# matteofox/MC-ALF

Measured on AMD Instinct MI355X. Metric: component-pixel Voigt evals/s (sum_s ncomp_s * npix / t), logL batch on MI355X: `value` with the inputs resident in HBM when the timed region starts, `value_host_api` through the host-pointer entry with P in and logL out inside every step, higher is better.
Workload: dtype f64

## Files before the change

mc-alf_amd/csrc/kernels.hip:

```cpp
#include <hip/hip_runtime.h>

#include <cmath>

#include "kernel_args.h"
#include "voigt_device.h"

namespace mcalf {

__device__ __forceinline__ int xcd_raw() { return (int)(__builtin_amdgcn_s_getreg((3 << 11) | 20) & 15); }
__device__ __forceinline__ int xcd_id() { return (int)(__builtin_amdgcn_s_getreg((3 << 11) | 20) & (kXcds - 1)); }

__device__ __forceinline__ int tile_pos(int i) { return (i & 7) * kPlaneStride + (i >> 3); }

template <int kCtrl, int kRowMask = 0xF>
__device__ __forceinline__ double dpp_move(double v) {
    const unsigned long long u = __builtin_bit_cast(unsigned long long, v);
    const int lo = __builtin_amdgcn_update_dpp(0, (int)(unsigned)u, kCtrl, kRowMask, 0xF, false);
    const int hi = __builtin_amdgcn_update_dpp(0, (int)(unsigned)(u >> 32), kCtrl, kRowMask, 0xF, false);
    return __builtin_bit_cast(double, ((unsigned long long)(unsigned)hi << 32) | (unsigned)lo);
}

__device__ __forceinline__ double wave_sum_to_last(double v) {
    v += dpp_move<0x111>(v);
    v += dpp_move<0x112>(v);
    v += dpp_move<0x114>(v);
    v += dpp_move<0x118>(v);
    v += dpp_move<0x142, 0xA>(v);
    v += dpp_move<0x143, 0xC>(v);
    return v;
}

__device__ __forceinline__ double wave_sum(double v) {
#pragma unroll
    for (int off = 32; off > 0; off >>= 1) v += __shfl_down(v, off, 64);
    return v;
}

__device__ __forceinline__ unsigned long long uniform64(unsigned long long v) {
    const unsigned lo = __builtin_amdgcn_readfirstlane((unsigned)v);
    const unsigned hi = __builtin_amdgcn_readfirstlane((unsigned)(v >> 32));
    return ((unsigned long long)hi << 32) | lo;
}

__device__ __forceinline__ double wave_allsum(double v) {
    const unsigned long long u = __builtin_bit_cast(unsigned long long, wave_sum_to_last(v));
    const unsigned lo = __builtin_amdgcn_readlane((unsigned)u, 63), hi = __builtin_amdgcn_readlane((unsigned)(u >> 32), 63);
    return __builtin_bit_cast(double, ((unsigned long long)hi << 32) | lo);
}

__device__ __forceinline__ double block_sum(double v, double* scratch, int tid) {
    v = wave_sum(v);
    if ((tid & 63) == 0) scratch[tid >> 6] = v;
    __syncthreads();
    double s = 0.0;
#pragma unroll
    for (int w = 0; w < kWaves; ++w) s += scratch[w];
    __syncthreads();
    return s;
}

__device__ __forceinline__ double finalize_value(int mode, double sum, double nnz, bool asymm, double c4,
                                                 double c5, double veto4, double veto5) {
    if (mode == kModeChi2) return (nnz == 0.0) ? INFINITY : sum;
    if (asymm && (c5 > veto5 || c4 > veto4)) return -INFINITY;
    return -0.5 * sum;
}

__device__ __noinline__ double pow10_edge(double x) { return pow(10.0, x); }
__device__ __forceinline__ double pow10_fast(double x) {
    constexpr double kLn10Hi = 2.302585092994045901, kLn10Lo = -2.1707562233822494e-16;
    if (!(fabs(x) <= 300.0)) return pow10_edge(x);
    const double p = x * kLn10Hi;
    const double e = fma(x, kLn10Hi, -p) + x * kLn10Lo;
    const double r = exp_neg(-p);
    return fma(r, e, r);
}

__device__ inline void build_line_record(double* rec, double logN, double z, double b_kms, const LineDev& ln,
                                         double dnu_seg) {
    const double cold = pow10_fast(logN);
    const double zp1 = z + 1.0;
    const double rdnu = ln.wrest_cm / (b_kms * 1e5);
    const double a = ln.gamma4pi * rdnu;
    const double cne = kTauConst * cold * ln.f;
    const double K = cne * rdnu;
    rec[0] = zp1 * rdnu;
    rec[1] = ln.nujk * rdnu;
    rec[2] = core_limit_x2(K);
    rec[3] = a;
    rec[4] = K;
    rec[5] = K * a * kInvSqrtPi;
    double flag = 0.0;
    if (!(a <= kYFastMax) || !(a >= 0.0)) flag = 1.0;
    else if (K * 1.6e-28 > 2e-17) flag = 1.0;
    rec[6] = 0.0;
    const float du = (float)(rec[0] * dnu_seg);
    const float du2 = du * du, du4 = du2 * du2;
    const float q = (float)(kInterpC / kInterpTol) * (float)rec[5] * du4 * du4;
    double uthr = (double)__builtin_amdgcn_exp2f(0.1f * __builtin_amdgcn_logf(fmaxf(q, 1.0f))) * 1.02;
    uthr = fmax(uthr, (double)__fsqrt_rn((float)rec[2]) * 1.000001);
    rec[7] = !(uthr < 1e30) ? INFINITY : uthr;
    if (flag != 0.0) {
        rec[2] = a; rec[3] = 0.0; rec[4] = 0.0; rec[5] = 0.0; rec[6] = K; rec[7] = 0.0;
    }
    if (!(fabs(zp1) < 1e100) && zp1 == zp1 && fabs(K) < 1e100 && fabs(a) < 1e100) {
        rec[0] = 0.0; rec[1] = -1e6; rec[2] = 36.0; rec[3] = 0.0; rec[4] = 0.0; rec[5] = 0.0; rec[6] = 0.0;
        rec[7] = 0.0;
    }
}

__device__ __forceinline__ void fmac_inplace(double& acc, double a, double b) {
    asm("v_fmac_f64 %0, %1, %2" : "+v"(acc) : "v"(a), "v"(b));
}
__device__ __forceinline__ void add_inplace(double& acc, double a) {
    asm("v_add_f64 %0, %0, %1" : "+v"(acc) : "v"(a));
}

__device__ __forceinline__ void eval_line(const double* __restrict__ tab,
                                          const double (&nu)[kPpt], double (&tau)[kPpt], double nuNode,
                                          double& farNode, unsigned long long segOk) {
    const double A = tab[kLineLds + 1], B = tab[kLineLds + 2];
    double cF[VT_FDEG + 1];
#pragma unroll
    for (int k = 0; k <= VT_FDEG; ++k) cF[k] = tab[kZFLds + k];
    unsigned long long done = 0;
    if (kFarInterp) {
        const double uthr = tab[kLineLds];
        const double un = fma(nuNode, A, -B);
        const double x2n = un * un;
        const double t = fast_rcp(fmax(x2n, 4.0));
        unsigned long long mp = __builtin_amdgcn_ballot_w64(un >= uthr);
        unsigned long long mn = __builtin_amdgcn_ballot_w64(un <= -uthr);
        mp &= mp >> 7;
        mn &= mn >> 7;
        done = uniform64((mp | mn) & segOk);
        if (done != 0) {
            const unsigned long long lanes = ((unsigned long long)((unsigned)(done >> 32) * 0xFFu) << 32) | ((unsigned)done * 0xFFu);
            const bool mine = __builtin_amdgcn_inverse_ballot_w64(lanes);
            double P;
            if (!mine || x2n >= kX2Far) {
                P = cF[VT_FDEG];
#pragma unroll
                for (int k = VT_FDEG - 1; k >= 0; --k) P = fma(P, t, cF[k]);
            } else {
                const bool z0 = x2n >= kX2Wing;
                const double sv = z0 ? t : fma(t, VT_Z1_A, VT_Z1_B);
                const double* cw = tab + (z0 ? kZ0Lds : VT_Z1_OFF);
                P = cw[VT_WDEG];
#pragma unroll
                for (int k = VT_WDEG - 1; k >= 0; --k) P = fma(P, sv, cw[k]);
            }
            fmac_inplace(farNode, mine ? t : 0.0, P);
        }
    }
    const unsigned doneLo = (unsigned)done, doneHi = (unsigned)(done >> 32);
#pragma unroll
    for (int h = 0; h < kPpt / 4; ++h) {
    const unsigned dh = h ? doneHi : doneLo;
    if (dh == 0x01010101u) continue;
#pragma unroll
    for (int jj = 0; jj < 4; ++jj) {
        const int j = 4 * h + jj;
        if (__builtin_expect(((dh >> (8 * jj)) & 1u) != 0u, 1)) continue;
        const double u = fma(nu[j], A, -B);
        const double x2 = u * u;
        double t, P;
        if (x2 >= kX2Far) {
            t = fast_rcp(x2);
            P = cF[VT_FDEG];
#pragma unroll
            for (int k = VT_FDEG - 1; k >= 0; --k) P = fma(P, t, cF[k]);
        } else if (x2 >= kX2Wing) {
            t = fast_rcp(x2);
            const double* cw = tab + kZ0Lds;
            P = cw[VT_WDEG];
#pragma unroll
            for (int k = VT_WDEG - 1; k >= 0; --k) P = fma(P, t, cw[k]);
        } else {
            const double x4 = fabs(u) * 4.0;
            const int jx = (int)x4;
            const double sv = fma(x4, 2.0, -(double)(2 * jx + 1));
            const double* cc = tab + jx * VT_CSTRIDE;
            P = cc[VT_CDEG];
#pragma unroll
            for (int k = VT_CDEG - 1; k >= 0; --k) P = fma(P, sv, cc[k]);
            t = 1.0;
        }
        fmac_inplace(tau[j], t, P);
    }
    }
}

__device__ __forceinline__ double sample_param(const KArgs& a, const double* __restrict__ p, int i) {
    double v = p[i];
    if (a.prior_lo) {
        const double lo = a.prior_lo[i], hi = a.prior_hi[i];
        {
#pragma clang fp contract(off)
            const double scaled = v * (hi - lo);
            v = scaled + lo;
        }
        if (a.prior_int && i == a.startind) v = trunc(v);
    }
    return v;
}

constexpr int kOrderBuckets = 64;
constexpr int kOrderKeys = 16;

template <bool kZeroPad>
__device__ __forceinline__ int sample_ncomp(const KArgs& a, long s) {
    const double ncv = sample_param(a, a.P + (size_t)s * a.ndim, a.startind);
    const double nct = kZeroPad ? floor(ncv) : trunc(ncv);
    return (nct >= 1.0) ? ((nct >= (double)a.ncompmax) ? a.ncompmax : (int)nct) : 0;
}

template <bool kZeroPad>
__device__ void build_order(const KArgs& a, long batch) {
    __shared__ int hist[kOrderBuckets];
    const int tid = threadIdx.x, nthr = blockDim.x;
    if (tid < kOrderBuckets) hist[tid] = 0;
    __syncthreads();
    const long chunk = (long)kOrderKeys * nthr;
    auto load_keys = [&](long base, int (&key)[kOrderKeys]) {
#pragma unroll
        for (int k = 0; k < kOrderKeys; ++k) {
            const long s = base + (long)k * nthr + tid;
            key[k] = (s < batch) ? min(a.ncompmax - sample_ncomp<kZeroPad>(a, s), kOrderBuckets - 1) : -1;
        }
    };
    int key[kOrderKeys];
    for (long base = 0; base < batch; base += chunk) {
        load_keys(base, key);
#pragma unroll
        for (int k = 0; k < kOrderKeys; ++k)
            if (key[k] >= 0) atomicAdd(&hist[key[k]], 1);
    }
    __syncthreads();
    if (tid < 64) {
        static_assert(kOrderBuckets == 64, "one bucket per lane");
        const int c = hist[tid];
        int incl = c;
#pragma unroll
        for (int off = 1; off < 64; off <<= 1) {
            const int up = __shfl_up(incl, off, 64);
            if (tid >= off) incl += up;
        }
        hist[tid] = incl - c;
    }
    __syncthreads();
    for (long base = 0; base < batch; base += chunk) {
        if (batch > chunk) load_keys(base, key);
#pragma unroll
        for (int k = 0; k < kOrderKeys; ++k)
            if (key[k] >= 0) a.order[atomicAdd(&hist[key[k]], 1)] = (int)(base + (long)k * nthr + tid);
    }
}

template <bool kZeroPad>
__device__ __forceinline__ void setup_sample(const KArgs& a, long s, int lane, double* recs, double* taps, bool writeTaps,
                                             SampleHdr* hdrOut, bool writeTheta) {
    const int rowlen = (a.mode == kModeOneComp) ? 5 : a.ndim;
    const double* p = a.P + (size_t)s * rowlen;
    double R, cont;
    int nc, nfill_eff;
    if (a.mode == kModeOneComp) {
        R = p[0];
        cont = p[1];
        nc = 1;
        nfill_eff = 0;
    } else {
        R = a.freespecres ? sample_param(a, p, 0) : a.specres_fixed;
        cont = a.freecont ? sample_param(a, p, a.freespecres ? 1 : 0) : a.contval_fixed;
        const double ncv = sample_param(a, p, a.startind);
        if (a.theta_out && writeTheta)
            for (int i = lane; i < a.ndim; i += 64) a.theta_out[(size_t)s * a.ndim + i] = sample_param(a, p, i);
        const double nct = kZeroPad ? floor(ncv) : trunc(ncv);
        nc = (nct >= 1.0) ? ((nct >= (double)a.ncompmax) ? a.ncompmax : (int)nct) : 0;
        nfill_eff = a.targonly ? 0 : a.nfill;
    }
    const int nl_eff = (a.mode == kModeOneComp && a.onecomp_fill) ? 1 : a.nlines;
    const int ncl = nc * nl_eff + nfill_eff;

    const int nTargetSlots = (a.mode == kModeOneComp) ? nl_eff : a.ncompmax * a.nlines;
    const int nSlots = nTargetSlots + ((a.mode == kModeOneComp) ? 0 : a.nfill);
    int ngenLane = 0;
    for (int slot = lane; slot < nSlots; slot += 64) {
        double logN, z, b;
        const LineDev* ln;
        int dst;
        if (a.mode == kModeOneComp) {
            logN = p[2]; z = p[3]; b = p[4];
            ln = (a.onecomp_fill == 0) ? (a.lines + slot)
               : (a.onecomp_fill == 1) ? (a.lines + a.nlines) : (a.lines + (a.onecomp_fill - 2));
            dst = slot;
        } else if (slot < nTargetSlots) {
            const int c = slot / a.nlines;
            const int l = slot - c * a.nlines;
            const int q = 1 + 3 * c + a.startind;
            logN = sample_param(a, p, q); z = sample_param(a, p, q + 1); b = sample_param(a, p, q + 2);
            ln = a.lines + l;
            dst = (c < nc) ? slot : -1;
        } else {
            const int k = slot - nTargetSlots;
            const int q = 3 * k + a.endind;
            logN = sample_param(a, p, q); z = sample_param(a, p, q + 1); b = sample_param(a, p, q + 2);
            ln = a.lines + a.nlines;
            dst = (nfill_eff > 0) ? nc * a.nlines + k : -1;
        }
        double rec[kRecStride];
        build_line_record(rec, logN, z, b, *ln, a.dnu_seg);
        ngenLane += __popcll(__ballot(dst >= 0 && rec[6] != 0.0));
        if (dst >= 0) {
#pragma unroll
            for (int k = 0; k < kRecStride; ++k) recs[dst * kRecStride + k] = rec[k];
        }
    }

    int n;
    bool bad = false;
    const double sigma = (R / kFwhmToSigma) / a.velstep;
    if (kZeroPad) {
        n = a.jax_half;
    } else if (R > a.velstep) {
        const double nd = ceil(kKernelReach * sigma);
        if (!(nd <= (double)a.n_cap)) { bad = true; n = 0; }
        else n = (int)nd;
    } else {
        n = 0;
    }
    const int ntap8 = (2 * n + 1 + 7) & ~7;
    const double inv2s2 = kZeroPad ? 1.0 / (2.0 * sigma * sigma) : 0.5 / (sigma * sigma);
    const double amp = kZeroPad ? 1.0 : 1.0 / (sqrt(2.0 * M_PI) * sigma);
    double wsum = 0.0, botOrdered = 0.0;
    if (ntap8 <= 64) {
        const double dk = (double)(lane - n);
        const double g = (lane > 2 * n) ? 0.0 : ((n == 0 && !kZeroPad) ? 1.0 : exp_neg((dk * dk) * inv2s2) * amp);
        const double gsum = wave_allsum(g);
        wsum = g / gsum;
        if (lane < ntap8 && writeTaps) taps[lane] = wsum;
        if (!kZeroPad) {
            const unsigned long long wb = __builtin_bit_cast(unsigned long long, wsum);
            const int last = __builtin_amdgcn_readfirstlane(2 * n);
#pragma unroll
            for (int k = 0; k < 64; ++k) {
                if (k <= last) {
                    const unsigned lo = __builtin_amdgcn_readlane((unsigned)wb, k), hi = __builtin_amdgcn_readlane((unsigned)(wb >> 32), k);
                    botOrdered += __builtin_bit_cast(double, ((unsigned long long)hi << 32) | lo);
                }
            }
        }
    } else {
        double gsum = 0.0;
        for (int k = lane; k <= 2 * n; k += 64) {
            const double dk = (double)(k - n);
            gsum += exp_neg((dk * dk) * inv2s2) * amp;
        }
        gsum = wave_allsum(gsum);
        for (int k = lane; k < ntap8; k += 64) {
            const double dk = (double)(k - n);
            const double w = (k <= 2 * n) ? exp_neg((dk * dk) * inv2s2) * amp / gsum : 0.0;
            if (writeTaps) taps[k] = w;
        }
        if (!kZeroPad)
            for (int k = 0; k <= 2 * n; ++k) {
                const double dk = (double)(k - n);
                botOrdered += exp_neg((dk * dk) * inv2s2) * amp / gsum;
            }
    }
    const double bot = kZeroPad ? 1.0 : botOrdered;
    const int ngen = ngenLane;
    if (lane == 0) {
        SampleHdr h;
        h.cont = cont; h.bot = bot; h.ncl = ncl; h.n = n; h.bad = bad ? 1 : 0; h.ngeneral = ngen;
        *hdrOut = h;
    }
}

__device__ __forceinline__ void stream_stores_done() { asm volatile("s_waitcnt vmcnt(0)" ::: "memory"); }
__device__ __forceinline__ void stream_compiler_barrier() { asm volatile("" ::: "memory"); }

__device__ __forceinline__ bool stream_gave_up(const KArgs& a) {
    return __hip_atomic_load(a.status, __ATOMIC_RELAXED, __HIP_MEMORY_SCOPE_SYSTEM) != 0u;
}

__device__ __forceinline__ bool stream_wait_arrived(const KArgs& a, unsigned r, unsigned& seen) {
    if (seen > r) return true;
    const unsigned long long t0 = __builtin_amdgcn_s_memrealtime();
    while (true) {
        seen = __hip_atomic_load(a.arrived, __ATOMIC_RELAXED, __HIP_MEMORY_SCOPE_SYSTEM);
        stream_compiler_barrier();
        if (seen > r) return true;
        if ((long long)(__builtin_amdgcn_s_memrealtime() - t0) > a.spin_ticks || stream_gave_up(a)) {
            __hip_atomic_store(a.status, kStreamHostLate, __ATOMIC_RELAXED, __HIP_MEMORY_SCOPE_SYSTEM);
            return false;
        }
        __builtin_amdgcn_s_sleep(32);
    }
}

__device__ __forceinline__ void stream_wait_ready(const KArgs& a, int s, unsigned early) {
    if (early != a.gen) {
        const unsigned long long t0 = __builtin_amdgcn_s_memrealtime();
        while (__hip_atomic_load(a.ready + s, __ATOMIC_RELAXED, __HIP_MEMORY_SCOPE_AGENT) != a.gen) {
            if ((long long)(__builtin_amdgcn_s_memrealtime() - t0) > a.spin_ticks) {
                __hip_atomic_store(a.status, kStreamStampLate, __ATOMIC_RELAXED, __HIP_MEMORY_SCOPE_SYSTEM);
                break;
            }
            __builtin_amdgcn_s_sleep(4);
        }
    }
    stream_compiler_barrier();
}

template <bool kZeroPad>
__global__ __launch_bounds__(kSetupBlockMax) void mcalf_sample_kernel(const KArgs a, long batch) {
    int blk = blockIdx.x;
    if (a.order) {
        if (blk == 0) { build_order<kZeroPad>(a, batch); return; }
        --blk;
    }
    const long s = (long)blk * (blockDim.x >> 6) + (threadIdx.x >> 6);
    if (s >= batch) return;
    const int lane = threadIdx.x & 63;
    if (s == 0 && lane == 0) *a.queue = 0u;
    setup_sample<kZeroPad>(a, s, lane, a.recs + (size_t)s * a.ncl_cap * kRecStride,
                           a.taps + (a.taps_shared ? 0 : (size_t)s * (2 * a.n_cap + 8)), !a.taps_shared || s == 0, a.hdr + s, true);
}

__device__ __forceinline__ void eval_general_lines(const double* __restrict__ sRec, int ncl, const double (&nu)[kPpt],
                                                double (&tau)[kPpt]) {
    for (int cl = 0; cl < ncl; ++cl) {
        const double* rec = sRec + cl * kRecStride;
        if (rec[6] == 0.0) continue;
        const double A = rec[0], B = rec[1], y = rec[2], K = rec[6];
#pragma unroll 1
        for (int j = 0; j < kPpt; ++j) {
            const double u = fma(nu[j], A, -B);
            tau[j] = fma(K, hjert_general(fabs(u), y), tau[j]);
        }
    }
}

template <bool kZeroPad>
__device__ __forceinline__ void stream_setup_phase(const KArgs& a, int tid, int x, int* sClaim) {
    const int lane = tid & 63, wave = tid >> 6;
    constexpr int nx = kXcds;
    const int nloc = stream_rows_of(a.nrows, x, nx), nblk = (nloc + 7) >> 3;
    const int eager = min(a.eager_rows, nblk);
    KArgs as = a;
    if (a.Pdev) as.P = a.Pdev;
    unsigned seen = a.arrived ? 0u : (unsigned)a.nrows;
    if (tid == 0) sClaim[3] = (int)atomicAdd(&a.sctl->arrive[x], 1u);
    __syncthreads();
    const bool dedicated = sClaim[3] < a.stream_wgs;
    bool rest = false;
    __builtin_amdgcn_s_setprio(3);
    while (true) {
        if (tid == 0) {
            const int want = rest ? max(a.rest_chunk >> 3, 1) : 1, lim = rest ? nblk : eager;
            const int c = rest ? eager + (int)atomicAdd(&a.sctl->sq_rest[x], (unsigned)want) : (int)atomicAdd(&a.sctl->sq_eager[x], 1u);
            const int cnt = c < lim ? min(want, lim - c) : 0;
            int ok = 1;
            if (cnt != 0 && a.arrived) {
                const int last = min(stream_row(x, 8 * (c + cnt) - 1, nx), a.nrows - 1);
                ok = stream_wait_arrived(a, (unsigned)last, seen) ? 1 : 0;
            }
            sClaim[0] = c; sClaim[1] = cnt; sClaim[2] = ok;
        }
        __syncthreads();
        const int c = sClaim[0], cnt = sClaim[1];
        const bool ok = sClaim[2] != 0;
        __syncthreads();
        if (cnt == 0) {
            if (!rest && dedicated) { rest = true; continue; }
            break;
        }
        if (a.Pdev && ok) {
            const int perBlock = 8 * a.ndim, n = cnt * perBlock;
            for (int i0 = tid; i0 < n; i0 += 4 * kBlock) {
                double v[4];
                size_t at[4];
#pragma unroll
                for (int k = 0; k < 4; ++k) {
                    const int i = i0 + k * kBlock, blk = i / perBlock;
                    at[k] = (size_t)stream_row(x, 8 * (c + blk), nx) * a.ndim + (size_t)(i - blk * perBlock);
                    v[k] = (i < n && at[k] < (size_t)a.nrows * a.ndim) ? a.P[at[k]] : 0.0;
                }
#pragma unroll
                for (int k = 0; k < 4; ++k)
                    if (i0 + k * kBlock < n && at[k] < (size_t)a.nrows * a.ndim) a.Pdev[at[k]] = v[k];
            }
            stream_stores_done();
            __syncthreads();
        }
        for (int k = 0; k < cnt; ++k) {
            const int r = stream_row(x, 8 * (c + k) + wave, nx);
            if (r >= a.nrows) continue;
            SampleHdr* hdrp = reinterpret_cast<SampleHdr*>(reinterpret_cast<double*>(a.hdr) + (size_t)r * a.hdr_stride);
            if (ok) {
                setup_sample<kZeroPad>(as, (long)r, lane, a.recs + (size_t)r * a.rec_stride, a.taps + (size_t)r * a.tap_stride, true, hdrp, true);
            } else if (lane == 0) {
                SampleHdr h;
                h.cont = 0.0; h.bot = 1.0; h.ncl = 0; h.n = 0; h.bad = 1; h.ngeneral = 0;
                *hdrp = h;
            }
        }
        stream_stores_done();
        if (lane < cnt) {
            const int r = stream_row(x, 8 * (c + lane) + wave, nx);
            if (r < a.nrows) __hip_atomic_store(a.ready + r, a.gen, __ATOMIC_RELAXED, __HIP_MEMORY_SCOPE_AGENT);
        }
    }
    __builtin_amdgcn_s_setprio(0);
    __syncthreads();
}

__device__ __forceinline__ void stream_exit(const KArgs& a, int tid) {
    if (tid != 0) return;
    stream_stores_done();
    if (atomicAdd(&a.sctl->exited, 1u) == gridDim.x - 1) {
        unsigned lo = ~0u, hi = 0u;
        for (int k = 0; k < kXcds; ++k) {
            const unsigned n = __hip_atomic_load(&a.sctl->arrive[k], __ATOMIC_RELAXED, __HIP_MEMORY_SCOPE_AGENT);
            lo = min(lo, n); hi = max(hi, n);
        }
        __hip_atomic_store(a.status + 2, lo, __ATOMIC_RELAXED, __HIP_MEMORY_SCOPE_SYSTEM);
        __hip_atomic_store(a.status + 3, hi, __ATOMIC_RELAXED, __HIP_MEMORY_SCOPE_SYSTEM);
        for (int k = 0; k < kXcds; ++k) {
            __hip_atomic_store(&a.sctl->arrive[k], 0u, __ATOMIC_RELAXED, __HIP_MEMORY_SCOPE_AGENT);
            __hip_atomic_store(&a.sctl->sq_eager[k], 0u, __ATOMIC_RELAXED, __HIP_MEMORY_SCOPE_AGENT);
            __hip_atomic_store(&a.sctl->sq_rest[k], 0u, __ATOMIC_RELAXED, __HIP_MEMORY_SCOPE_AGENT);
            __hip_atomic_store(&a.sctl->queue[k], 0u, __ATOMIC_RELAXED, __HIP_MEMORY_SCOPE_AGENT);
        }
        __hip_atomic_store(&a.sctl->exited, 0u, __ATOMIC_RELAXED, __HIP_MEMORY_SCOPE_AGENT);
        stream_stores_done();
        __hip_atomic_store(a.status + 1, a.gen, __ATOMIC_RELAXED, __HIP_MEMORY_SCOPE_SYSTEM);
    }
}

struct ItemLoads {
    double treg[(VT_NY * VT_NTOT + kBlock - 1) / kBlock];
    double rreg[2];
    double tapreg;
    double nu[kPpt];
    double nuNode;
    unsigned long long tileMask;
    SampleHdr hd;
};

template <bool kZeroPad, bool selfHalo, bool kInline, bool kCoh = false>
__device__ __forceinline__ void request_item(const KArgs& a, int w, int tid, ItemLoads& L) {
    asm volatile("" : "+v"(tid));
    constexpr int kTRegs = (VT_NY * VT_NTOT + kBlock - 1) / kBlock;
    constexpr int kRecRegs = 2;
    const int recTotal = a.ncl_cap * kRecStride, tapTotal = 2 * a.n_cap + 8;
    const int s = w / a.ntiles;
    const int tileIdx = w - s * a.ntiles;
#pragma unroll
    for (int i = 0; i < kTRegs; ++i) {
        const int idx = tid + i * kBlock;
        L.treg[i] = (idx < VT_NY * VT_NTOT) ? a.tabs[idx] : 0.0;
    }
    if (!kInline) {
        const double* gr = a.recs + (size_t)s * (kCoh ? a.rec_stride : recTotal);
        const double* gt = a.taps + (kCoh ? (size_t)s * a.tap_stride : (a.taps_shared ? 0 : (size_t)s * tapTotal));
        L.hd = kCoh ? *reinterpret_cast<const SampleHdr*>(reinterpret_cast<const double*>(a.hdr) + (size_t)s * a.hdr_stride) : a.hdr[s];
#pragma unroll
        for (int i = 0; i < kRecRegs; ++i) L.rreg[i] = (tid + i * kBlock < recTotal) ? gr[tid + i * kBlock] : 0.0;
        L.tapreg = (tid < tapTotal) ? gt[tid] : 0.0;
    }
    const int t0 = tileIdx * a.tile;
    const int ext0 = selfHalo ? 0 : t0 - a.n_cap;
    int npixW = a.npix;
    asm volatile("" : "+s"(npixW));
#pragma unroll
    for (int j = 0; j < kPpt; ++j) {
        int e = ext0 + tid + j * kBlock;
        if (!selfHalo && (e < 0 || e >= a.npix)) {
            if (kZeroPad) e = 0;
            else { e %= npixW; if (e < 0) e += npixW; }
        }
        L.nu[j] = a.nu[e];
    }
    L.nuNode = 0.0;
    L.tileMask = 0;
    if (kFarInterp) {
        const int wv = tid >> 6, ln = tid & 63;
        int e = ext0 + 64 * wv + kBlock * (ln >> 3) + VT_INTERP_NODES[ln & 7];
        if (!selfHalo && (e < 0 || e >= a.npix)) { e %= npixW; if (e < 0) e += npixW; }
        L.nuNode = a.nu[e];
        L.tileMask = a.segok[tileIdx];
    }
}

template <bool kZeroPad, bool kSelfHalo, int kLinesPerSync, bool kInline, bool kStream>
__device__ __forceinline__ void fused_items(const KArgs& a, double* smem) {
    double* sTab = smem;
    double* sRec = sTab + 2 * kLinesPerSync * kTabPad;
    double* sW = sRec + a.ncl_cap * kRecStride;
    double* sRed = sW + (2 * a.n_cap + 8);
    double* sWt = sRed + kRedDoubles;
    double* sF = sWt + 64 * VT_INODES;
    int* sNext = reinterpret_cast<int*>(sRed + 3 * kWaves);

    const int tid0 = threadIdx.x;
    double* sT = sF;
    constexpr int kTRegs = (VT_NY * VT_NTOT + kBlock - 1) / kBlock;
    constexpr int kRecRegs = 2;
    constexpr bool selfHalo = kSelfHalo;
    if (kFarInterp) sWt[(tid0 & 7) * 64 + (tid0 >> 3)] = a.wtab[tid0];
    const int recTotal = a.ncl_cap * kRecStride, tapTotal = 2 * a.n_cap + 8;
    const int xcd = kStream ? xcd_id() : 0;
    const int nItems = kStream ? stream_rows_of(a.nrows, xcd, kXcds) * a.ntiles : a.nitems;

    constexpr bool kOrdered = kSelfHalo && !kInline && !kStream;
    auto item_of = [&](int t) -> int {
        if (kStream) { const int j = t / a.ntiles; return stream_row(xcd, j, kXcds) * a.ntiles + (t - j * a.ntiles); }
        return (kOrdered && a.order) ? a.order[t] : t;
    };
    constexpr bool kDeferTicket = kOrdered || kStream;
    int w;
    unsigned int* const queue = kStream ? &a.sctl->queue[xcd] : a.queue;
    const int firstTickets = kStream ? 0 : (int)gridDim.x;
    if (kStream) {
        if (tid0 == 0) sNext[0] = (int)atomicAdd(queue, 1u);
        __syncthreads();
        const int t = sNext[0];
        __syncthreads();
        if (t >= nItems) {
            stream_exit(a, tid0);
            return;
        }
        w = item_of(t);
        stream_wait_ready(a, w / a.ntiles, 0u);
    } else {
        w = item_of(blockIdx.x);
    }
    ItemLoads L;
    request_item<kZeroPad, kSelfHalo, kInline, kStream>(a, w, tid0, L);

    while (true) {
        int tid = tid0;
        asm volatile("" : "+v"(tid));
        const bool hasCoef = tid < VT_NTOT;
        const int coefPos = tid + (tid >= VT_Z0_OFF ? 1 : 0) + (tid >= VT_ZF_OFF ? 1 : 0);
        const bool coreCoef = tid < VT_NCORE;
        const int s = w / a.ntiles;
        const int tileIdx = w - s * a.ntiles;
        const int t0 = tileIdx * a.tile;
        const int tlen = min(a.tile, a.npix - t0);
        const int ext0 = selfHalo ? 0 : t0 - a.n_cap;
        const int extCount = tlen + 2 * a.n_cap;
        double nu[kPpt], tau[kPpt];
#pragma unroll
        for (int j = 0; j < kPpt; ++j) {
            const int idx = tid + j * kBlock;
            const int e = ext0 + idx;
            const bool zero = kZeroPad && !selfHalo && (e < 0 || e >= a.npix);
            nu[j] = L.nu[j];
            tau[j] = (zero && idx < extCount) ? INFINITY : 0.0;
        }
        const double nuNode = L.nuNode;
        double farNode = 0.0;
        unsigned long long segOk = 0;
        if (kFarInterp) {
            const int wv = tid >> 6;
#pragma unroll
            for (int j = 0; j < kPpt; ++j) segOk |= ((L.tileMask >> (wv + 8 * j)) & 1ULL) << (8 * j);
            segOk = uniform64(segOk);
        }
        SampleHdr hd;
        SampleHdr* sHdr = reinterpret_cast<SampleHdr*>(sRed + 2 * kWaves);
        static_assert(sizeof(SampleHdr) <= kWaves * sizeof(double), "header fits the scratch slot");
        if (kInline) {
            if (tid < 64) setup_sample<kZeroPad>(a, s, tid, sRec, sW, true, sHdr, tileIdx == 0);
        } else {
            hd = L.hd;
#pragma unroll
            for (int i = 0; i < kRecRegs; ++i)
                if (tid + i * kBlock < recTotal) sRec[tid + i * kBlock] = L.rreg[i];
            if (recTotal > kRecRegs * kBlock) {
                const double* gr = a.recs + (size_t)s * (kStream ? a.rec_stride : recTotal);
                for (int i = tid + kRecRegs * kBlock; i < recTotal; i += kBlock) sRec[i] = gr[i];
            }
            if (tid < tapTotal) sW[tid] = L.tapreg;
            if (tapTotal > kBlock) {
                const double* gt = a.taps + (kStream ? (size_t)s * a.tap_stride : (a.taps_shared ? 0 : (size_t)s * tapTotal));
                for (int i = tid + kBlock; i < tapTotal; i += kBlock) sW[i] = gt[i];
            }
        }
#pragma unroll
        for (int i = 0; i < kTRegs; ++i) {
            const int idx = tid + i * kBlock;
            if (idx < VT_NY * VT_NTOT) sT[idx] = L.treg[i];
        }
        int tHeld = nItems, wHeld = 0;
        unsigned stHeld = 0u;
        if (tid == 0) {
            tHeld = a.persist ? firstTickets + (int)atomicAdd(queue, 1u) : nItems;
            if (kOrdered) wHeld = (tHeld < nItems) ? item_of(tHeld) : 0;
            else if (kStream) {
                wHeld = (tHeld < nItems) ? item_of(tHeld) : 0;
                if (tHeld < nItems) stHeld = __hip_atomic_load(a.ready + wHeld / a.ntiles, __ATOMIC_RELAXED, __HIP_MEMORY_SCOPE_AGENT);
            } else { sNext[0] = tHeld; sNext[1] = tHeld; }
        }

        __syncthreads();
        if (kInline) hd = *sHdr;
        const double cont = kStream ? __builtin_bit_cast(double, uniform64(__builtin_bit_cast(unsigned long long, hd.cont))) : hd.cont;
        const double bot = kStream ? __builtin_bit_cast(double, uniform64(__builtin_bit_cast(unsigned long long, hd.bot))) : hd.bot;
        const int ncl = kStream ? min(max(hd.ncl, 0), a.ncl_cap) : hd.ncl, n = kStream ? min(max(hd.n, 0), a.n_cap) : hd.n;
        const bool bad = hd.bad != 0;
        const int shift = a.n_cap - n;
        int tNext = 0, wNext = 0;
        if (!kDeferTicket) {
            tNext = __builtin_amdgcn_readfirstlane(sNext[0]);
            wNext = __builtin_amdgcn_readfirstlane(sNext[1]);
        }
        int buf = 0;
        const int ncl_run = ncl;
        for (int cl0 = 0; cl0 < ncl_run; cl0 += kLinesPerSync) {
            if (4 * cl0 < ncl_run) __builtin_amdgcn_s_setprio(3);
            else if (4 * cl0 < 2 * ncl_run) __builtin_amdgcn_s_setprio(2);
            else if (4 * cl0 < 3 * ncl_run) __builtin_amdgcn_s_setprio(1);
            else __builtin_amdgcn_s_setprio(0);
            double* tabs = sTab + buf * (kLinesPerSync * kTabPad);
            if (hasCoef) {
                double Tn[VT_NY];
#pragma unroll
                for (int nn = 0; nn < VT_NY; ++nn) Tn[nn] = sT[nn * VT_NTOT + tid];
                double fy[kLinesPerSync], fs[kLinesPerSync], fc[kLinesPerSync];
#pragma unroll
                for (int l = 0; l < kLinesPerSync; ++l) {
                    const double* rec = sRec + min(cl0 + l, ncl_run - 1) * kRecStride;
                    fy[l] = rec[3];
                    fs[l] = coreCoef ? rec[4] : rec[5];
                    fc[l] = Tn[VT_NY - 1];
                }
#pragma unroll
                for (int nn = VT_NY - 2; nn >= 0; --nn) {
#pragma unroll
                    for (int l = 0; l < kLinesPerSync; ++l) fc[l] = fma(fc[l], fy[l], Tn[nn]);
                    __builtin_amdgcn_sched_barrier(0);
                }
#pragma unroll
                for (int l = 0; l < kLinesPerSync; ++l) tabs[l * kTabPad + coefPos] = fc[l] * fs[l];
            } else if (tid >= kBlock - 64 && tid < kBlock - 64 + 3) {
                const int which = tid - (kBlock - 64);
                const int src = (which == 0) ? 7 : which - 1;
#pragma unroll
                for (int l = 0; l < kLinesPerSync; ++l)
                    tabs[l * kTabPad + kLineLds + which] = sRec[min(cl0 + l, ncl_run - 1) * kRecStride + src];
            }
            __syncthreads();
            buf ^= 1;
            const int lmax = __builtin_amdgcn_readfirstlane(min(kLinesPerSync, ncl_run - cl0));
#pragma unroll 1
            for (int l = 0; l < lmax; ++l) eval_line(tabs + l * kTabPad, nu, tau, nuNode, farNode, segOk);
        }
        if (hd.ngeneral > 0 && ncl_run > 0) eval_general_lines(sRec, ncl, nu, tau);
        __builtin_amdgcn_s_setprio(0);
        double wrow[VT_INODES];
        double* sFar = sTab + (tid >> 6) * 64;
        if (kFarInterp) {
            __syncthreads();
            sFar[tid & 63] = farNode;
#pragma unroll
            for (int k = 0; k < VT_INODES; ++k) wrow[k] = sWt[k * 64 + (tid & 63)];
        }
        const int extTight = tlen + 2 * n;
        const int posBody = tile_pos(selfHalo ? tid + n : tid - shift);
        const int posLow = tile_pos(tid + n + a.npix), posHigh = tile_pos(tid + n - a.npix);
        static_assert(kBlock % 8 == 0, "tile_pos(i + kBlock) == tile_pos(i) + kBlock / 8");
        static_assert(kPpt % 2 == 0, "pixels are processed in pairs");
#pragma unroll
        for (int j0 = 0; j0 < kPpt; j0 += 2) {
            double fl[2];
#pragma unroll
            for (int jj = 0; jj < 2; ++jj) {
                const int j = j0 + jj;
                double tj = tau[j];
                if (kFarInterp) {
                    double add = 0.0;
#pragma unroll
                    for (int k = 0; k < VT_INODES; ++k) add = fma(wrow[k], sFar[8 * j + k], add);
                    tj += add;
                }
                fl[jj] = exp_neg(tj);
            }
#pragma unroll
            for (int jj = 0; jj < 2; ++jj) {
                const int j = j0 + jj;
                if (selfHalo) {
                    const int p = tid + j * kBlock;
                    if (p < a.npix) {
                        sF[posBody + (kBlock / 8) * j] = fl[jj];
                        if (j * kBlock < n && p < n) sF[posLow + (kBlock / 8) * j] = kZeroPad ? 0.0 : fl[jj];
                        if ((j + 1) * kBlock > a.npix - n && p >= a.npix - n) sF[posHigh + (kBlock / 8) * j] = kZeroPad ? 0.0 : fl[jj];
                    }
                } else {
                    const int pos = tid + j * kBlock - shift;
                    if (pos >= 0 && pos < extTight) sF[posBody + (kBlock / 8) * j] = fl[jj];
                }
            }
            __builtin_amdgcn_sched_barrier(0);
            asm volatile("" ::: "memory");
        }
        if (tid < kTileSlack) {
            double zero = 0.0;
            asm volatile("" : "+v"(zero));
            sF[tile_pos(extTight + tid)] = zero;
        }
        if (kDeferTicket && tid == 0) { sNext[0] = tHeld; sNext[1] = wHeld; if (kStream) sNext[2] = (int)stHeld; }
        __syncthreads();
        if (kDeferTicket) {
            tNext = __builtin_amdgcn_readfirstlane(sNext[0]);
            wNext = __builtin_amdgcn_readfirstlane(sNext[1]);
        }
        unsigned stampNext = 0u;
        if (kStream) stampNext = (unsigned)__builtin_amdgcn_readfirstlane(sNext[2]);

        double acc = 0.0, nnz = 0.0, c4 = 0.0, c5 = 0.0;
        const int base = 8 * tid;
        const bool reduces = (a.mode == kModeLogL || a.mode == kModeChi2);
        if (base < tlen) {
            const size_t o0 = (size_t)(t0 + base);
            double ob[8], is2[8], lg[8];
#pragma unroll
            for (int m = 0; m < 8; ++m) { ob[m] = a.obj[o0 + m]; is2[m] = a.ispec2[o0 + m]; lg[m] = a.lgis[o0 + m]; }
            double win[8], top[8];
            const double* fp = sF + tid;
#pragma unroll
            for (int m = 0; m < 8; ++m) { win[m] = fp[m * kPlaneStride]; top[m] = 0.0; }
            const double* wp = sW;
            const int ntaps = 2 * n + 1;
            for (int q0 = 0; q0 + 8 <= ntaps; q0 += 8) {
                ++fp;
#pragma unroll
                for (int r = 0; r < 8; ++r) {
                    const double wgt = wp[r];
#pragma unroll
                    for (int m = 0; m < 8; ++m) top[m] = fma(win[(m + r) & 7], wgt, top[m]);
                    win[r] = fp[r * kPlaneStride];
                }
                wp += 8;
            }
            {
                const int rem = ntaps & 7;
                ++fp;
#pragma unroll
                for (int r = 0; r < 7; ++r) {
                    if (r >= rem) break;
                    const double wgt = wp[r];
#pragma unroll
                    for (int m = 0; m < 8; ++m) top[m] = fma(win[(m + r) & 7], wgt, top[m]);
                    win[r] = fp[r * kPlaneStride];
                }
            }
            const double ibot = 1.0 / bot;
            const bool plainLogL = !kZeroPad && a.mode == kModeLogL && !a.asymm && a.model == nullptr;
            if (plainLogL) {
                if (!bad) {
#pragma unroll
                    for (int m = 0; m < 8; ++m) {
                        double mval = top[m] * ibot;
                        mval *= cont;
                        const double d = ob[m] - mval;
                        double term = is2[m] * (d * d);
                        term = (term - lg[m]) + a.log2pi;
                        acc += (base + m < tlen && !isnan(term)) ? term : 0.0;
                    }
                }
            } else if (!kZeroPad && a.mode != kModeLogL && a.mode != kModeChi2 && a.model != nullptr) {
                double* mrow = a.model + (size_t)s * a.npix + t0 + base;
#pragma unroll
                for (int m = 0; m < 8; ++m) {
                    double mval = top[m] * ibot;
                    mval *= cont;
                    if (bad) mval = NAN;
                    if (base + m < tlen) mrow[m] = mval;
                }
            } else
#pragma unroll
            for (int m = 0; m < 8; ++m) {
                const int i = base + m;
                const bool live = i < tlen;
                const int pix = t0 + i;
                double mval = kZeroPad ? top[m] : top[m] * ibot;
                if (kZeroPad && (pix < n || pix >= a.npix - n)) mval = sF[tile_pos(min(i, tlen - 1) + n)];
                mval *= cont;
                if (bad) mval = NAN;
                if (a.model && live) a.model[(size_t)s * a.npix + pix] = mval;
                if (reduces) {
                    const double d = ob[m] - mval;
                    double term = is2[m] * (d * d);
                    if (a.mode == kModeLogL) term = (term - lg[m]) + a.log2pi;
                    if (live && !isnan(term)) acc += term;
                    if (a.mode == kModeChi2 && live && mval != 0.0) nnz += 1.0;
                    if (a.asymm) {
                        const double resid = d / a.err[o0 + m];
                        if (live && resid > 4.0) c4 += 1.0;
                        if (live && resid > 5.0) c5 += 1.0;
                    }
                }
            }
        }
        const bool more = tNext < nItems;
        __builtin_amdgcn_sched_barrier(0);
        if (kStream && more) stream_wait_ready(a, wNext / a.ntiles, stampNext);
        if (!kInline) request_item<kZeroPad, kSelfHalo, kInline, kStream>(a, more ? wNext : w, tid, L);
        __builtin_amdgcn_sched_barrier(0);
        if (reduces) {
            acc = wave_sum_to_last(acc);
            if (a.mode == kModeChi2) nnz = wave_sum_to_last(nnz);
            const int wave = tid >> 6;
            if ((tid & 63) == 63) { sRed[wave] = acc; sRed[kWaves + wave] = nnz; }
        }
        double t4 = 0.0, t5 = 0.0;
        if (reduces && a.asymm) {
            __syncthreads();
            t4 = block_sum(c4, sRed + 2 * kWaves, tid);
            t5 = block_sum(c5, sRed + 2 * kWaves, tid);
        }
        __syncthreads();
        if (reduces && tid == 0) {
            double ssum = 0.0, scnt = 0.0;
#pragma unroll
            for (int wv = 0; wv < kWaves; ++wv) { ssum += sRed[wv]; scnt += sRed[kWaves + wv]; }
            if (bad) { ssum = INFINITY; scnt = 1.0; }
            if (a.ntiles == 1) {
                const double val = finalize_value(a.mode, ssum, scnt, a.asymm != 0, t4, t5, a.veto4, a.veto5);
                if (kStream || kInline) __hip_atomic_store(a.out + s, val, __ATOMIC_RELAXED, __HIP_MEMORY_SCOPE_SYSTEM);
                else a.out[s] = val;
            } else {
                double* pr = a.partial + ((size_t)s * a.ntiles + tileIdx) * 4;
                pr[0] = ssum; pr[1] = scnt; pr[2] = t4; pr[3] = t5;
            }
        }
        if (kInline || !more) break;
        w = wNext;
    }
    if (kStream) stream_exit(a, tid0);
}

template <bool kZeroPad, bool kSelfHalo, int kLinesPerSync, bool kInline, bool kStream>
__global__ __launch_bounds__(kBlock, kMinWaves) void mcalf_fused_kernel(const KArgs a) {
    static_assert(!(kInline && kStream), "the one-launch variant of small calls has no queue to stream through");
    extern __shared__ __align__(16) double smem[];
    if constexpr (kStream) {
        stream_setup_phase<kZeroPad>(a, threadIdx.x, xcd_id(), reinterpret_cast<int*>(smem));

        typedef __attribute__((address_space(4))) const KArgs ArgSeg;
        ArgSeg* kp = (ArgSeg*)__builtin_amdgcn_kernarg_segment_ptr();
        asm volatile("" : "+s"(kp));
        KArgs fresh = *(const KArgs*)kp;
        fused_items<kZeroPad, kSelfHalo, kLinesPerSync, kInline, kStream>(fresh, smem);
    } else {
        fused_items<kZeroPad, kSelfHalo, kLinesPerSync, kInline, kStream>(a, smem);
    }
}

template <bool kZeroPad, bool kSelfHalo>
__global__ __launch_bounds__(kBlock, 2) void mcalf_resident_kernel(const KArgs a, ResidentBox* boxes, ResidentShared* shared,
                                                                           long long idle_ticks, int row_offset_doubles) {
    extern __shared__ __align__(16) double smem[];
    double* sRow = smem + row_offset_doubles;
    unsigned* sCtl = reinterpret_cast<unsigned*>(sRow + kResRowMax);
    const int tid = threadIdx.x;
    ResidentBox* box = boxes + blockIdx.x;
    const unsigned long long t_launch = __builtin_amdgcn_s_memrealtime();
    unsigned seen = __hip_atomic_load(&box->ack, __ATOMIC_RELAXED, __HIP_MEMORY_SCOPE_SYSTEM);
    while (true) {
        if (tid == 0) {
            unsigned r;
            while (true) {
                const unsigned long long both = __hip_atomic_load(reinterpret_cast<unsigned long long*>(&box->req), __ATOMIC_RELAXED,
                                                                   __HIP_MEMORY_SCOPE_SYSTEM);
                r = (unsigned)both;
                if (r != seen) break;
                bool leave = (unsigned)(both >> 32) != 0u || __hip_atomic_load(&shared->leave, __ATOMIC_RELAXED, __HIP_MEMORY_SCOPE_AGENT) != 0u;
                if (!leave && blockIdx.x == 0) {
                    const unsigned long long last = __hip_atomic_load(&shared->last, __ATOMIC_RELAXED, __HIP_MEMORY_SCOPE_AGENT);
                    const unsigned long long since = last > t_launch ? last : t_launch;
                    if ((long long)(__builtin_amdgcn_s_memrealtime() - since) > idle_ticks) leave = true;
                }
                if (leave) {
                    __hip_atomic_store(&shared->leave, 1u, __ATOMIC_RELAXED, __HIP_MEMORY_SCOPE_AGENT);
                    __hip_atomic_store(&box->state, kResLeaving, __ATOMIC_RELAXED, __HIP_MEMORY_SCOPE_SYSTEM);
                    stream_stores_done();
                    r = __hip_atomic_load(&box->req, __ATOMIC_RELAXED, __HIP_MEMORY_SCOPE_SYSTEM);
                    if (r != seen) { __hip_atomic_store(&box->state, kResRunning, __ATOMIC_RELAXED, __HIP_MEMORY_SCOPE_SYSTEM); break; }
                    __hip_atomic_store(&box->state, kResGone, __ATOMIC_RELAXED, __HIP_MEMORY_SCOPE_SYSTEM);
                    break;
                }
                __builtin_amdgcn_s_sleep(2);
            }
            sCtl[0] = r;
        }
        __syncthreads();
        const unsigned r = sCtl[0];
        __syncthreads();
        if (r == seen) return;
        if (tid < kResRowMax) {
            const unsigned long long bits = __hip_atomic_load(reinterpret_cast<unsigned long long*>(box->row) + tid, __ATOMIC_RELAXED,
                                                               __HIP_MEMORY_SCOPE_SYSTEM);
            sRow[tid] = __builtin_bit_cast(double, bits);
        }
        __syncthreads();
        typedef __attribute__((address_space(4))) const KArgs ArgSeg;
        ArgSeg* kp = (ArgSeg*)__builtin_amdgcn_kernarg_segment_ptr();
        asm volatile("" : "+s"(kp));
        KArgs b = *(const KArgs*)kp;
        const int rowlen = b.ndim;
        b.P = sRow - (size_t)blockIdx.x * rowlen;
        b.out = &box->result - blockIdx.x;
        fused_items<kZeroPad, kSelfHalo, 4, true, false>(b, smem);
        if (tid == 0) {
            stream_stores_done();
            __hip_atomic_store(&box->ack, r, __ATOMIC_RELAXED, __HIP_MEMORY_SCOPE_SYSTEM);
            __hip_atomic_fetch_max(&shared->last, __builtin_amdgcn_s_memrealtime(), __ATOMIC_RELAXED, __HIP_MEMORY_SCOPE_AGENT);
        }
        seen = r;
        __syncthreads();
    }
}

__global__ void mcalf_finalize_kernel(const double* partial, double* out, long batch, int ntiles, int mode,
                                      int asymm, double veto4, double veto5, unsigned int* fin_count, unsigned int* done_word,
                                      unsigned int gen) {
    const long s = (long)blockIdx.x * blockDim.x + threadIdx.x;
    if (s < batch) {
        double sum = 0.0, cnt = 0.0, c4 = 0.0, c5 = 0.0;
        for (int t = 0; t < ntiles; ++t) {
            const double* pr = partial + (s * ntiles + t) * 4;
            sum += pr[0]; cnt += pr[1]; c4 += pr[2]; c5 += pr[3];
        }
        const double val = finalize_value(mode, sum, cnt, asymm != 0, c4, c5, veto4, veto5);
        if (done_word) __hip_atomic_store(out + s, val, __ATOMIC_RELAXED, __HIP_MEMORY_SCOPE_SYSTEM);
        else out[s] = val;
    }
    if (done_word) {
        stream_stores_done();
        __syncthreads();
        if (threadIdx.x == 0 && atomicAdd(fin_count, 1u) == gridDim.x - 1) {
            __hip_atomic_store(fin_count, 0u, __ATOMIC_RELAXED, __HIP_MEMORY_SCOPE_AGENT);
            stream_stores_done();
            __hip_atomic_store(done_word, gen, __ATOMIC_RELAXED, __HIP_MEMORY_SCOPE_SYSTEM);
        }
    }
}

__global__ void mcalf_hjert_kernel(const double* x, const double* y, long n, double* out, const double* tabs,
                                   int node_form) {
    const long i = (long)blockIdx.x * blockDim.x + threadIdx.x;
    if (i < n) out[i] = hjert_folded(x[i], y[i], tabs, node_form != 0);
}

__global__ void mcalf_scale_cube_kernel(const double* lo, const double* hi, const double* cube, long total,
                                        int ndim, int slot, int int_ncomp, double* theta) {
    const long i = (long)blockIdx.x * blockDim.x + threadIdx.x;
    if (i >= total) return;
    const int d = (int)(i % ndim);
    double v;
    {
#pragma clang fp contract(off)
        const double scaled = cube[i] * (hi[d] - lo[d]);
        v = scaled + lo[d];
    }
    if (int_ncomp && d == slot) v = trunc(v);
    theta[i] = v;
}

constexpr int kWideBlock = kWideBlockThreads;
constexpr int kWidePlane = (kWideBlockPix + kWideTapChunk + 16) / 8 + 2;
static_assert(kWideBlockPix == 8 * kWideBlock && kWideTapChunk % 8 == 0 && kWidePlane % 32 == 4, "wide convolution geometry");
__device__ __forceinline__ int wide_pos(int i) { return (i & 7) * kWidePlane + (i >> 3); }
__device__ __forceinline__ double wide_block_sum(double v, double* red, int tid) {
    v = wave_sum(v);
    if ((tid & 63) == 0) red[tid >> 6] = v;
    __syncthreads();
    double s = 0.0;
#pragma unroll
    for (int w = 0; w < kWideBlock / 64; ++w) s += red[w];
    __syncthreads();
    return s;
}

__device__ __forceinline__ void wide_decode(const KArgs& a, long s, double& R, double& cont) {
    const int rowlen = (a.mode == kModeOneComp) ? 5 : a.ndim;
    const double* p = a.P + (size_t)s * rowlen;
    if (a.mode == kModeOneComp) { R = p[0]; cont = p[1]; return; }
    R = a.freespecres ? sample_param(a, p, 0) : a.specres_fixed;
    cont = a.freecont ? sample_param(a, p, a.freespecres ? 1 : 0) : a.contval_fixed;
}

template <bool kZeroPad>
__global__ __launch_bounds__(kWideBlock) void mcalf_wide_taps_kernel(const KArgs a, double* taps, long tap_stride, SampleHdr* hdr) {
    __shared__ double red[kWideBlock / 64];
    const long s = blockIdx.x;
    const int tid = threadIdx.x;
    double R, cont;
    wide_decode(a, s, R, cont);
    const double sigma = (R / kFwhmToSigma) / a.velstep;
// ... 186 lines not shown
```

Before: 605.4 billion.

## Precompute per-line far-wing segment masks at setup instead of per-tile ballots

During per-sample setup, each line record now gets a 64-bit mask, stored in the threshold slot, that marks which 64-pixel segments lie wholly in the far wing. The fused kernel's self-halo path reads this mask to skip pixels and node evaluation, replacing the per-line ballot and threshold test in the inner loop. The node-sum layout in LDS also changes to reuse the idle half of the folded table buffer, and interpolation-node frequencies are loaded directly for the self-halo case. This shifts work into setup, which now does a serial loop over lines with readlanes, and it relies on the nu grid and segok layout assumptions matching.

```diff
diff --git a/mc-alf_amd/csrc/kernels.hip b/mc-alf_amd/csrc/kernels.hip
--- a/mc-alf_amd/csrc/kernels.hip
+++ b/mc-alf_amd/csrc/kernels.hip
@@ -116,15 +116,44 @@
     asm("v_add_f64 %0, %0, %1" : "+v"(acc) : "v"(a));
 }
 
+template <bool kPreMask>
 __device__ __forceinline__ void eval_line(const double* __restrict__ tab,
                                           const double (&nu)[kPpt], double (&tau)[kPpt], double nuNode,
-                                          double& farNode, unsigned long long segOk) {
+                                          double& farNode, unsigned long long segOk, int wv) {
     const double A = tab[kLineLds + 1], B = tab[kLineLds + 2];
     double cF[VT_FDEG + 1];
 #pragma unroll
     for (int k = 0; k <= VT_FDEG; ++k) cF[k] = tab[kZFLds + k];
+    auto node_pass = [&](unsigned long long done, double x2n, double t) {
+        const unsigned long long lanes = ((unsigned long long)((unsigned)(done >> 32) * 0xFFu) << 32) | ((unsigned)done * 0xFFu);
+        const bool mine = __builtin_amdgcn_inverse_ballot_w64(lanes);
+        double P;
+        if (!mine || x2n >= kX2Far) {
+            P = cF[VT_FDEG];
+#pragma unroll
+            for (int k = VT_FDEG - 1; k >= 0; --k) P = fma(P, t, cF[k]);
+        } else {
+            const bool z0 = x2n >= kX2Wing;
+            const double sv = z0 ? t : fma(t, VT_Z1_A, VT_Z1_B);
+            const double* cw = tab + (z0 ? kZ0Lds : VT_Z1_OFF);
+            P = cw[VT_WDEG];
+#pragma unroll
+            for (int k = VT_WDEG - 1; k >= 0; --k) P = fma(P, sv, cw[k]);
+        }
+        fmac_inplace(farNode, mine ? t : 0.0, P);
+    };
     unsigned long long done = 0;
-    if (kFarInterp) {
+    unsigned pix = 0;
+    if (kFarInterp && kPreMask) {
+        const unsigned long long W = uniform64(__builtin_bit_cast(unsigned long long, tab[kLineLds]));
+        pix = (unsigned)(W >> (8 * wv)) & 0xFFu;
+        const unsigned long long nodes = (W >> wv) & 0x0101010101010101ull;
+        if (nodes != 0) {
+            const double un = fma(nuNode, A, -B);
+            const double x2n = un * un;
+            node_pass(nodes, x2n, fast_rcp(fmax(x2n, 4.0)));
+        }
+    } else if (kFarInterp) {
         const double uthr = tab[kLineLds];
         const double un = fma(nuNode, A, -B);
         const double x2n = un * un;
@@ -134,34 +163,17 @@
         mp &= mp >> 7;
         mn &= mn >> 7;
         done = uniform64((mp | mn) & segOk);
-        if (done != 0) {
-            const unsigned long long lanes = ((unsigned long long)((unsigned)(done >> 32) * 0xFFu) << 32) | ((unsigned)done * 0xFFu);
-            const bool mine = __builtin_amdgcn_inverse_ballot_w64(lanes);
-            double P;
-            if (!mine || x2n >= kX2Far) {
-                P = cF[VT_FDEG];
-#pragma unroll
-                for (int k = VT_FDEG - 1; k >= 0; --k) P = fma(P, t, cF[k]);
-            } else {
-                const bool z0 = x2n >= kX2Wing;
-                const double sv = z0 ? t : fma(t, VT_Z1_A, VT_Z1_B);
-                const double* cw = tab + (z0 ? kZ0Lds : VT_Z1_OFF);
-                P = cw[VT_WDEG];
-#pragma unroll
-                for (int k = VT_WDEG - 1; k >= 0; --k) P = fma(P, sv, cw[k]);
-            }
-            fmac_inplace(farNode, mine ? t : 0.0, P);
-        }
+        if (done != 0) node_pass(done, x2n, t);
     }
     const unsigned doneLo = (unsigned)done, doneHi = (unsigned)(done >> 32);
 #pragma unroll
     for (int h = 0; h < kPpt / 4; ++h) {
     const unsigned dh = h ? doneHi : doneLo;
-    if (dh == 0x01010101u) continue;
+    if (kPreMask ? ((pix >> (4 * h)) & 0xFu) == 0xFu : dh == 0x01010101u) continue;
 #pragma unroll
     for (int jj = 0; jj < 4; ++jj) {
         const int j = 4 * h + jj;
-        if (__builtin_expect(((dh >> (8 * jj)) & 1u) != 0u, 1)) continue;
+        if (__builtin_expect((kPreMask ? (pix >> j) & 1u : (dh >> (8 * jj)) & 1u) != 0u, 1)) continue;
         const double u = fma(nu[j], A, -B);
         const double x2 = u * u;
         double t, P;
@@ -257,11 +269,36 @@
     }
 }
 
+__device__ __forceinline__ double readlane_f64(double v, int lane) {
+    const unsigned long long u = __builtin_bit_cast(unsigned long long, v);
+    const unsigned lo = __builtin_amdgcn_readlane((unsigned)u, lane), hi = __builtin_amdgcn_readlane((unsigned)(u >> 32), lane);
+    return __builtin_bit_cast(double, ((unsigned long long)hi << 32) | lo);
+}
+
+__device__ __forceinline__ double segment_masks(const double (&rec)[kRecStride], int lane, unsigned long long have, double nuLo,
+                                                double nuHi, unsigned long long okW) {
+    unsigned long long word = 0;
+    for (unsigned long long todo = have; todo != 0; todo &= todo - 1) {
+        const int r = __builtin_ctzll(todo);
+        const double A = readlane_f64(rec[0], r), B = readlane_f64(rec[1], r), uthr = readlane_f64(rec[7], r);
+        const double u0 = fma(nuLo, A, -B), u1 = fma(nuHi, A, -B);
+        const unsigned long long mp = __builtin_amdgcn_ballot_w64(u0 >= uthr) & __builtin_amdgcn_ballot_w64(u1 >= uthr);
+        const unsigned long long mn = __builtin_amdgcn_ballot_w64(u0 <= -uthr) & __builtin_amdgcn_ballot_w64(u1 <= -uthr);
+        const unsigned long long w = (mp | mn) & okW;
+        if (lane == r) word = w;
+    }
+    return __builtin_bit_cast(double, word);
+}
+
 template <bool kZeroPad>
 __device__ __forceinline__ void setup_sample(const KArgs& a, long s, int lane, double* recs, double* taps, bool writeTaps,
-                                             SampleHdr* hdrOut, bool writeTheta) {
+                                             SampleHdr* hdrOut, bool writeTheta, bool segMasks) {
     const int rowlen = (a.mode == kModeOneComp) ? 5 : a.ndim;
     const double* p = a.P + (size_t)s * rowlen;
+    const int mseg = 8 * (lane & 7) + (lane >> 3);
+    double nuLo = 0.0, nuHi = 0.0;
+    unsigned long long tileOk = 0;
+    if (segMasks) { nuLo = a.nu[64 * mseg]; nuHi = a.nu[64 * mseg + 63]; tileOk = a.segok[0]; }
     double R, cont;
     int nc, nfill_eff;
     if (a.mode == kModeOneComp) {
@@ -285,7 +322,10 @@
     const int nTargetSlots = (a.mode == kModeOneComp) ? nl_eff : a.ncompmax * a.nlines;
     const int nSlots = nTargetSlots + ((a.mode == kModeOneComp) ? 0 : a.nfill);
     int ngenLane = 0;
-    for (int slot = lane; slot < nSlots; slot += 64) {
+    const int nSlotsRun = segMasks ? (nSlots + 63) & ~63 : nSlots;
+    for (int slot0 = lane; slot0 < nSlotsRun; slot0 += 64) {
+        const bool spare = segMasks && slot0 >= nSlots;
+        const int slot = spare ? nSlots - 1 : slot0;
         double logN, z, b;
         const LineDev* ln;
         int dst;
@@ -308,8 +348,12 @@
             ln = a.lines + a.nlines;
             dst = (nfill_eff > 0) ? nc * a.nlines + k : -1;
         }
+        if (spare) dst = -1;
         double rec[kRecStride];
         build_line_record(rec, logN, z, b, *ln, a.dnu_seg);
+        if (segMasks)
+            rec[7] = segment_masks(rec, lane, __builtin_amdgcn_ballot_w64(dst >= 0), nuLo, nuHi,
+                                   __builtin_amdgcn_ballot_w64(((tileOk >> mseg) & 1ULL) != 0));
         ngenLane += __popcll(__ballot(dst >= 0 && rec[6] != 0.0));
         if (dst >= 0) {
 #pragma unroll
@@ -425,7 +469,8 @@
     const int lane = threadIdx.x & 63;
     if (s == 0 && lane == 0) *a.queue = 0u;
     setup_sample<kZeroPad>(a, s, lane, a.recs + (size_t)s * a.ncl_cap * kRecStride,
-                           a.taps + (a.taps_shared ? 0 : (size_t)s * (2 * a.n_cap + 8)), !a.taps_shared || s == 0, a.hdr + s, true);
+                           a.taps + (a.taps_shared ? 0 : (size_t)s * (2 * a.n_cap + 8)), !a.taps_shared || s == 0, a.hdr + s, true,
+                           a.selfhalo != 0);
 }
 
 __device__ __forceinline__ void eval_general_lines(const double* __restrict__ sRec, int ncl, const double (&nu)[kPpt],
@@ -442,7 +487,7 @@
     }
 }
 
-template <bool kZeroPad>
+template <bool kZeroPad, bool kSelfHalo>
 __device__ __forceinline__ void stream_setup_phase(const KArgs& a, int tid, int x, int* sClaim) {
     const int lane = tid & 63, wave = tid >> 6;
     constexpr int nx = kXcds;
@@ -499,7 +544,8 @@
             if (r >= a.nrows) continue;
             SampleHdr* hdrp = reinterpret_cast<SampleHdr*>(reinterpret_cast<double*>(a.hdr) + (size_t)r * a.hdr_stride);
             if (ok) {
-                setup_sample<kZeroPad>(as, (long)r, lane, a.recs + (size_t)r * a.rec_stride, a.taps + (size_t)r * a.tap_stride, true, hdrp, true);
+                setup_sample<kZeroPad>(as, (long)r, lane, a.recs + (size_t)r * a.rec_stride, a.taps + (size_t)r * a.tap_stride, true, hdrp, true,
+                                       kSelfHalo);
             } else if (lane == 0) {
                 SampleHdr h;
                 h.cont = 0.0; h.bot = 1.0; h.ncl = 0; h.n = 0; h.bad = 1; h.ngeneral = 0;
@@ -585,7 +631,10 @@
     }
     L.nuNode = 0.0;
     L.tileMask = 0;
-    if (kFarInterp) {
+    if (kFarInterp && selfHalo && !kInline) {
+        const int wv = tid >> 6, ln = tid & 63;
+        L.nuNode = a.nu[kBlock * wv + 64 * (ln >> 3) + VT_INTERP_NODES[ln & 7]];
+    } else if (kFarInterp) {
         const int wv = tid >> 6, ln = tid & 63;
         int e = ext0 + 64 * wv + kBlock * (ln >> 3) + VT_INTERP_NODES[ln & 7];
         if (!selfHalo && (e < 0 || e >= a.npix)) { e %= npixW; if (e < 0) e += npixW; }
@@ -609,6 +658,8 @@
     constexpr int kTRegs = (VT_NY * VT_NTOT + kBlock - 1) / kBlock;
     constexpr int kRecRegs = 2;
     constexpr bool selfHalo = kSelfHalo;
+    constexpr bool kPreMask = kSelfHalo && !kInline;
+    static_assert(kLinesPerSync * kTabPad >= kBlock, "the node sums fit the idle half of the folded tables");
     if (kFarInterp) sWt[(tid0 & 7) * 64 + (tid0 >> 3)] = a.wtab[tid0];
     const int recTotal = a.ncl_cap * kRecStride, tapTotal = 2 * a.n_cap + 8;
     const int xcd = kStream ? xcd_id() : 0;
@@ -664,17 +715,18 @@
         const double nuNode = L.nuNode;
         double farNode = 0.0;
         unsigned long long segOk = 0;
-        if (kFarInterp) {
+        if (kFarInterp && !kPreMask) {
             const int wv = tid >> 6;
 #pragma unroll
             for (int j = 0; j < kPpt; ++j) segOk |= ((L.tileMask >> (wv + 8 * j)) & 1ULL) << (8 * j);
             segOk = uniform64(segOk);
         }
+        const int wvU = kPreMask ? __builtin_amdgcn_readfirstlane(tid >> 6) : 0;
         SampleHdr hd;
         SampleHdr* sHdr = reinterpret_cast<SampleHdr*>(sRed + 2 * kWaves);
         static_assert(sizeof(SampleHdr) <= kWaves * sizeof(double), "header fits the scratch slot");
         if (kInline) {
-            if (tid < 64) setup_sample<kZeroPad>(a, s, tid, sRec, sW, true, sHdr, tileIdx == 0);
+            if (tid < 64) setup_sample<kZeroPad>(a, s, tid, sRec, sW, true, sHdr, tileIdx == 0, false);
         } else {
             hd = L.hd;
 #pragma unroll
@@ -757,15 +809,17 @@
             buf ^= 1;
             const int lmax = __builtin_amdgcn_readfirstlane(min(kLinesPerSync, ncl_run - cl0));
 #pragma unroll 1
-            for (int l = 0; l < lmax; ++l) eval_line(tabs + l * kTabPad, nu, tau, nuNode, farNode, segOk);
+            for (int l = 0; l < lmax; ++l) eval_line<kPreMask>(tabs + l * kTabPad, nu, tau, nuNode, farNode, segOk, wvU);
         }
         if (hd.ngeneral > 0 && ncl_run > 0) eval_general_lines(sRec, ncl, nu, tau);
         __builtin_amdgcn_s_setprio(0);
         double wrow[VT_INODES];
-        double* sFar = sTab + (tid >> 6) * 64;
+        double* sFar = kPreMask ? sTab + buf * (kLinesPerSync * kTabPad) + 8 * (tid >> 6) : sTab + (tid >> 6) * 64;
+        constexpr int kFarSlot = kPreMask ? 64 : 8;
         if (kFarInterp) {
+            if (kPreMask) sTab[buf * (kLinesPerSync * kTabPad) + tid] = farNode;
             __syncthreads();
-            sFar[tid & 63] = farNode;
+            if (!kPreMask) sFar[tid & 63] = farNode;
 #pragma unroll
             for (int k = 0; k < VT_INODES; ++k) wrow[k] = sWt[k * 64 + (tid & 63)];
         }
@@ -784,7 +838,7 @@
                 if (kFarInterp) {
                     double add = 0.0;
 #pragma unroll
-                    for (int k = 0; k < VT_INODES; ++k) add = fma(wrow[k], sFar[8 * j + k], add);
+                    for (int k = 0; k < VT_INODES; ++k) add = fma(wrow[k], sFar[kFarSlot * j + k], add);
                     tj += add;
                 }
                 fl[jj] = exp_neg(tj);
@@ -949,7 +1003,7 @@
     static_assert(!(kInline && kStream), "the one-launch variant of small calls has no queue to stream through");
     extern __shared__ __align__(16) double smem[];
     if constexpr (kStream) {
-        stream_setup_phase<kZeroPad>(a, threadIdx.x, xcd_id(), reinterpret_cast<int*>(smem));
+        stream_setup_phase<kZeroPad, kSelfHalo>(a, threadIdx.x, xcd_id(), reinterpret_cast<int*>(smem));
 
         typedef __attribute__((address_space(4))) const KArgs ArgSeg;
         ArgSeg* kp = (ArgSeg*)__builtin_amdgcn_kernarg_segment_ptr();
```

After: 613.8 billion (median of 6 runs). 1.4% higher.
